# Byshx/Poccala

Measured on AMD Instinct MI355X. Metric: frames/sec GMM-score+fwd-bwd, 39-d MFCC, 2048-mix, higher is better.
Workload: dtype f32-class (f16x2 split operands, f32 accumulate; f64 dynamic programming)

## Files before the change

poccala_amd/csrc/gmm_score_split.hip:

```cpp
#include <stdlib.h>

#include "pcl_internal.h"

namespace {

#ifndef PCL_SPLIT_WG
#define PCL_SPLIT_WG 256
#endif
constexpr int WG = PCL_SPLIT_WG;
typedef float f16v __attribute__((ext_vector_type(16)));

#ifndef PCL_SPLIT16_NT
#define PCL_SPLIT16_NT 2
#endif
#ifndef PCL_SPLIT16_MINW
#define PCL_SPLIT16_MINW 3
#endif
#ifndef PCL_SPLIT16_MTS
#define PCL_SPLIT16_MTS 1
#endif
typedef _Float16 h8v __attribute__((ext_vector_type(8)));

template <int D, int NT>
__global__ __launch_bounds__(WG, PCL_SPLIT16_MINW * 256 / WG > 0 ? PCL_SPLIT16_MINW * 256 / WG : 1) void gmm_score_split16_kernel(
    const float *__restrict__ frames, const uint4 *__restrict__ pm, const float *__restrict__ fscale, const float *__restrict__ centers,
    int nmt_max, const ScoreTile *__restrict__ tiles, const ScoreSeg *__restrict__ segs, double *__restrict__ out,
    int *__restrict__ flags, const double *__restrict__ kzero, const int *__restrict__ n_on_pipe, const int *__restrict__ npt) {
    static_assert(D % 8 != 0, "the folded constants need a spare slot");
    constexpr int KS8 = (D + 7) / 8;
    constexpr int CH = 2 * KS8;
    constexpr int SC = D / 8, JC = D % 8;
    constexpr float FMAXH = 6.0e4f;
    const ScoreTile tile = tiles[blockIdx.x];
    const int lane = threadIdx.x & 63;
    const int wave = threadIdx.x >> 6;
    const int half = lane >> 5;
    const int col = lane & 31;
    if (tile.seg_lo >= tile.seg_hi) {
        if (threadIdx.x == 0) flags[blockIdx.x] = 0;
        return;
    }
    const int n_mtiles = npt[tile.state];
    __shared__ int s_ovf;
    if (threadIdx.x == 0) s_ovf = 0;
    __syncthreads();
    const int vend = segs[tile.seg_hi - 1].vstart + segs[tile.seg_hi - 1].len;
    const bool wave_active = tile.vstart + wave * NT * 32 < vend;
    if (n_mtiles == 0) {
        if (wave_active) {
            for (int c = 0; c < NT; ++c) {
                const int v = tile.vstart + (wave * NT + c) * 32 + col;
                if (v < vend && half == 0) {
                    int lo = tile.seg0;
                    const int hi = tile.seg_hi - 1;
                    while (lo < hi && segs[lo + 1].vstart <= v) ++lo;
                    const ScoreSeg sg = segs[lo];
                    out[sg.out0 + (long long)(v - sg.vstart) * sg.out_stride] = -INFINITY;
                }
            }
        }
        if (threadIdx.x == 0) flags[blockIdx.x] = 0;
        return;
    }

    h8v xb[NT][2][KS8];
    long long oidx[NT];
    bool valid[NT];
    const float *cen = centers + (size_t)tile.state * D;
    const float *fs = fscale + ((size_t)tile.state * 2 + half) * (KS8 * 8);
    bool ovf = false;
#pragma unroll
    for (int c = 0; c < NT; ++c) {
        int v = tile.vstart + (wave * NT + c) * 32 + col;
        valid[c] = v < vend;
        if (!valid[c]) v = tile.vstart;
        int lo = tile.seg0, hi = tile.seg_hi - 1;
        if (lo < hi && segs[lo + 1].vstart <= v) {
            ++lo;
            if (lo < hi && segs[lo + 1].vstart <= v) {
                ++lo;
                while (lo < hi) {
                    int mid = (lo + hi + 1) >> 1;
                    if (segs[mid].vstart <= v) lo = mid; else hi = mid - 1;
                }
            }
        }
        const ScoreSeg sg = segs[lo];
        const long long t = v - sg.vstart;
        const float *fp = frames + (sg.frame0 + t) * D;
#pragma unroll
        for (int s = 0; s < KS8; ++s)
#pragma unroll
            for (int j = 0; j < 8; ++j) {
                const int d = 8 * s + j;
                float val = 0.f;
                if (d < D) {
                    const float xc = fp[d] - cen[d];
                    val = (half ? xc : xc * xc) * fs[d];
                    ovf |= __builtin_fabsf(val) > FMAXH;
                    val = __builtin_fminf(__builtin_fmaxf(val, -FMAXH), FMAXH);
                }
                if (d == D) val = half ? 0.f : 1.f;
                const _Float16 h1 = (_Float16)val;
                xb[c][0][s][j] = h1;
                xb[c][1][s][j] = (_Float16)(val - (float)h1);
            }
        oidx[c] = sg.out0 + t * (long long)sg.out_stride;
    }
    if (__any(ovf) && lane == 0) s_ovf = 1;

    float sm[NT], ref[NT];
    bool inited[NT];
#pragma unroll
    for (int c = 0; c < NT; ++c) {
        sm[c] = 0.f;
        ref[c] = 0.f;
        inited[c] = false;
    }
    bool ref_ovf = false;

    constexpr int MTS = PCL_SPLIT16_MTS;
    __shared__ __attribute__((aligned(16))) uint4 abuf[2][MTS * CH * 64];
    const uint4 *pstate = pm + (size_t)tile.state * nmt_max * (CH * 64);
    auto dma = [&](int buf, int stage) {
        const uint4 *src = pstate + (size_t)stage * (MTS * CH * 64);
        const int nch = min(MTS, n_mtiles - stage * MTS) * CH;
        for (int p = wave; p < nch; p += WG / 64)
            __builtin_amdgcn_global_load_lds((const __attribute__((address_space(1))) void *)(src + p * 64 + lane),
                                             (__attribute__((address_space(3))) void *)&abuf[buf][p * 64], 16, 0, 0);
    };

#ifdef PCL_SPLIT_STAMPS
    unsigned long long st_acc[4] = {0, 0, 0, 0}, st_t = 0;
#define SSTAMP(k) { const unsigned long long t_ = __builtin_amdgcn_s_memtime(); st_acc[k] += t_ - st_t; st_t = t_; }
#else
#define SSTAMP(k)
#endif
    auto process = [&](int mt) {
        const uint4 *ab = &abuf[(mt / MTS) & 1][(mt % MTS) * (CH * 64)];
        f16v acc[NT];
#pragma unroll
        for (int c = 0; c < NT; ++c)
#pragma unroll
            for (int r = 0; r < 16; ++r) acc[c][r] = 0.f;
        auto pass = [&](int pa, int pb) {
#pragma unroll
            for (int s = 0; s < KS8; ++s) {
                const h8v a = *reinterpret_cast<const h8v *>(&ab[(pa * KS8 + s) * 64 + lane]);
#pragma unroll
                for (int c = 0; c < NT; ++c) acc[c] = __builtin_amdgcn_mfma_f32_32x32x16_f16(a, xb[c][pb][s], acc[c], 0, 0, 0);
            }
        };
#ifdef PCL_SPLIT_PRIO
        __builtin_amdgcn_s_setprio(1);
#endif
        pass(1, 0);
        pass(0, 1);
        pass(0, 0);
        SSTAMP(1)
#ifdef PCL_SPLIT_PRIO
        __builtin_amdgcn_s_setprio(0);
#endif
#ifdef PCL_DIAG_NOLSE
#pragma unroll
        for (int c = 0; c < NT; ++c) sm[c] += acc[c][0] + acc[c][15];
        return;
#endif
#pragma unroll
        for (int c = 0; c < NT; ++c) {
            float es[16];
#pragma unroll
            for (int r = 0; r < 16; ++r) es[r] = __builtin_amdgcn_exp2f(acc[c][r]);
#pragma unroll
            for (int w = 8; w >= 1; w >>= 1)
#pragma unroll
                for (int r = 0; r < w; ++r) es[r] += es[r + w];
            const float snew = sm[c] + es[0];
            if (__any(!inited[c]) || __any(!(snew < 3.0e38f))) {
                float gm = acc[c][0];
#pragma unroll
                for (int r = 1; r < 16; ++r) gm = __builtin_fmaxf(gm, acc[c][r]);
                const float gp = __builtin_fmaxf(gm, __shfl_xor(gm, 32, 64));
                float s = sm[c];
                const bool first = !inited[c];
                if ((first || gp > 0.f) && gp > -5.0e4f) {
                    const _Float16 r1 = (_Float16)__builtin_fminf(__builtin_fmaxf(-(ref[c] + gp), -FMAXH), FMAXH);
                    const float nref = -(float)r1, dl = nref - ref[c];
                    ref_ovf |= __builtin_fabsf(nref) > 5.0e4f;
#ifdef PCL_LSE_FLUSH_REPRO
                    s = first ? 0.f : s * __builtin_amdgcn_exp2f(-dl);
#else
                    const float hs = __builtin_amdgcn_exp2f(-0.5f * dl);
                    s = first ? 0.f : (s * hs) * hs;
#endif
                    inited[c] = true;
#pragma unroll
                    for (int r = 0; r < 16; ++r) acc[c][r] -= dl;
                    ref[c] = nref;
                    if (half) xb[c][0][SC][JC] = r1;
                }
#pragma unroll
                for (int r = 0; r < 16; ++r) s += __builtin_amdgcn_exp2f(acc[c][r]);
                sm[c] = s;
            } else {
                sm[c] = snew;
            }
        }
        SSTAMP(2)
    };
    const int n_stages = (n_mtiles + MTS - 1) / MTS;
    dma(0, 0);
#ifdef PCL_SPLIT_STAMPS
    st_t = __builtin_amdgcn_s_memtime();
#endif
    for (int st = 0; st < n_stages; ++st) {
        asm volatile("s_waitcnt vmcnt(0)" ::: "memory");
        SSTAMP(3)
        __syncthreads();
        SSTAMP(0)
        if (st == 0 && threadIdx.x == 0) flags[blockIdx.x] = s_ovf;
        if (st + 1 < n_stages) dma((st + 1) & 1, st + 1);
        if (wave_active) {
            const int mend = min(n_mtiles, (st + 1) * MTS);
            for (int mt = st * MTS; mt < mend; ++mt) process(mt);
        }
    }
#ifdef PCL_SPLIT_STAMPS
    if (blockIdx.x == 800 && lane == 0)
        printf("wave %d: per m-tile: dma-wait %llu  barrier %llu  dma-issue+lds+mfma %llu  lse %llu (memtime ticks)\n", wave,
               st_acc[3] / n_mtiles, st_acc[0] / n_mtiles, st_acc[1] / n_mtiles, st_acc[2] / n_mtiles);
#endif
    constexpr double LN2 = 0.693147180559945309417232121458;
    const double k0 = kzero[tile.state];
    if (wave_active && n_on_pipe[tile.state] > 0) {
#pragma unroll
        for (int c = 0; c < NT; ++c) ref_ovf |= !inited[c];
    }
#pragma unroll
    for (int c = 0; c < NT; ++c) {
        const double S = (double)sm[c] + (double)__shfl_xor(sm[c], 32, 64);
        if (valid[c] && half == 0) out[oidx[c]] = (S > 0) ? LN2 * ((double)ref[c] + k0 + ::log2(S)) : -INFINITY;
    }
    if (__any(ref_ovf) && lane == 0) s_ovf = 1;
    __syncthreads();
    if (threadIdx.x == 0 && s_ovf) flags[blockIdx.x] = 1;
}

template <int D>
void launch16_t(pcl_ctx *ctx, pcl_batch *b, const ScoreTile *tiles, int n_tiles) {
    constexpr size_t static_lds = 2 * (size_t)(2 * ((D + 7) / 8)) * 64 * 16;
    const size_t pad = (ctx->score_wgs_per_cu == 2 && static_lds < (56u << 10)) ? (56u << 10) - static_lds : 0;
    hipLaunchKernelGGL((gmm_score_split16_kernel<D, PCL_SPLIT16_NT>), dim3(n_tiles), dim3(WG), pad, ctx->stream, ctx->frames32,
                       reinterpret_cast<const uint4 *>(ctx->pm16f), ctx->fscale, ctx->centers32, ctx->Mpad32 / 32, tiles, b->d_segs,
                       b->Bt, b->d_tile_flags, ctx->kzero, ctx->d_non, ctx->d_npt);
}

}

int pcl_score_split16_tile_frames() { return WG / 64 * PCL_SPLIT16_NT * 32; }

int pcl_launch_score_split16(pcl_ctx *ctx, pcl_batch *b, const ScoreTile *tiles, int n_tiles) {
    if (n_tiles == 0) return PCL_OK;
    pcl_timer_begin(ctx, "score");
    switch (ctx->D) {
#define CASE(DD) case DD: launch16_t<DD>(ctx, b, tiles, n_tiles); break;
        PCL_MFMA_DIMS(CASE)
#undef CASE
        default: PCL_FAIL(ctx, PCL_ERR_INVALID, "internal: no split-f16 scoring kernel for D=%d", ctx->D);
    }
    pcl_timer_end(ctx, "score");
    HIPCHK(ctx, hipGetLastError());
    return PCL_OK;
}
```

Baseline: 20.75 million.

## Software-pipeline MFMA m-tiles with exp2 log-sum-exp of previous tile

Restructures the scoring loop so each step issues the MFMA chain for m-tile mt while computing exp2/log-sum-exp on the accumulators of m-tile mt-1, with sched_group_barrier interleaving MFMA and transcendental ops. It adds an optional 3-slot LDS ring using partial vmcnt waits and places the overflow flag inside the same LDS array. Launch-bounds min waves drops from 3 to 2, to make room for the doubled accumulator registers. The cost is higher VGPR pressure and lower occupancy, and the rescale path must now also shift the in-flight accumulator.

```diff
diff --git a/poccala_amd/csrc/gmm_score_split.hip b/poccala_amd/csrc/gmm_score_split.hip
--- a/poccala_amd/csrc/gmm_score_split.hip
+++ b/poccala_amd/csrc/gmm_score_split.hip
@@ -14,10 +14,13 @@
 #define PCL_SPLIT16_NT 2
 #endif
 #ifndef PCL_SPLIT16_MINW
-#define PCL_SPLIT16_MINW 3
-#endif
-#ifndef PCL_SPLIT16_MTS
-#define PCL_SPLIT16_MTS 1
+#define PCL_SPLIT16_MINW 2
+#endif
+#ifndef PCL_SPLIT16_RING
+#define PCL_SPLIT16_RING 2
+#endif
+#ifndef PCL_SPLIT16_TRANS_PER_MFMA
+#define PCL_SPLIT16_TRANS_PER_MFMA 1
 #endif
 typedef _Float16 h8v __attribute__((ext_vector_type(8)));
 
@@ -41,7 +44,9 @@
         return;
     }
     const int n_mtiles = npt[tile.state];
-    __shared__ int s_ovf;
+    constexpr int CHUNKS = 2 * ((D + 7) / 8);
+    __shared__ __attribute__((aligned(16))) uint4 lds[PCL_SPLIT16_RING * CHUNKS * 64 + 1];
+    int &s_ovf = *reinterpret_cast<int *>(&lds[PCL_SPLIT16_RING * CHUNKS * 64]);
     if (threadIdx.x == 0) s_ovf = 0;
     __syncthreads();
     const int vend = segs[tile.seg_hi - 1].vstart + segs[tile.seg_hi - 1].len;
@@ -119,67 +124,89 @@
     }
     bool ref_ovf = false;
 
-    constexpr int MTS = PCL_SPLIT16_MTS;
-    __shared__ __attribute__((aligned(16))) uint4 abuf[2][MTS * CH * 64];
+    constexpr int RING = PCL_SPLIT16_RING;
+    constexpr int NW = WG / 64;
+    uint4(*abuf)[CH * 64] = reinterpret_cast<uint4(*)[CH * 64]>(lds);
     const uint4 *pstate = pm + (size_t)tile.state * nmt_max * (CH * 64);
-    auto dma = [&](int buf, int stage) {
-        const uint4 *src = pstate + (size_t)stage * (MTS * CH * 64);
-        const int nch = min(MTS, n_mtiles - stage * MTS) * CH;
-        for (int p = wave; p < nch; p += WG / 64)
+    auto dma = [&](int slot, int mt) {
+        const uint4 *src = pstate + (size_t)mt * (CH * 64);
+        for (int p = wave; p < CH; p += NW)
             __builtin_amdgcn_global_load_lds((const __attribute__((address_space(1))) void *)(src + p * 64 + lane),
-                                             (__attribute__((address_space(3))) void *)&abuf[buf][p * 64], 16, 0, 0);
+                                             (__attribute__((address_space(3))) void *)&abuf[slot][p * 64], 16, 0, 0);
     };
-
-#ifdef PCL_SPLIT_STAMPS
-    unsigned long long st_acc[4] = {0, 0, 0, 0}, st_t = 0;
-#define SSTAMP(k) { const unsigned long long t_ = __builtin_amdgcn_s_memtime(); st_acc[k] += t_ - st_t; st_t = t_; }
-#else
-#define SSTAMP(k)
-#endif
-    auto process = [&](int mt) {
-        const uint4 *ab = &abuf[(mt / MTS) & 1][(mt % MTS) * (CH * 64)];
-        f16v acc[NT];
-#pragma unroll
-        for (int c = 0; c < NT; ++c)
-#pragma unroll
-            for (int r = 0; r < 16; ++r) acc[c][r] = 0.f;
-        auto pass = [&](int pa, int pb) {
-#pragma unroll
-            for (int s = 0; s < KS8; ++s) {
-                const h8v a = *reinterpret_cast<const h8v *>(&ab[(pa * KS8 + s) * 64 + lane]);
-#pragma unroll
-                for (int c = 0; c < NT; ++c) acc[c] = __builtin_amdgcn_mfma_f32_32x32x16_f16(a, xb[c][pb][s], acc[c], 0, 0, 0);
-            }
-        };
-#ifdef PCL_SPLIT_PRIO
-        __builtin_amdgcn_s_setprio(1);
-#endif
-        pass(1, 0);
-        pass(0, 1);
-        pass(0, 0);
-        SSTAMP(1)
-#ifdef PCL_SPLIT_PRIO
-        __builtin_amdgcn_s_setprio(0);
-#endif
-#ifdef PCL_DIAG_NOLSE
-#pragma unroll
-        for (int c = 0; c < NT; ++c) sm[c] += acc[c][0] + acc[c][15];
-        return;
-#endif
+    auto stage_ready = [&](int mt) {
+        if constexpr (RING == 2) {
+            asm volatile("s_waitcnt vmcnt(0)" ::: "memory");
+            __syncthreads();
+            if (mt + 1 < n_mtiles) dma((mt + 1) & 1, mt + 1);
+        } else {
+            constexpr int CHI = (CH + NW - 1) / NW, CLO = CH / NW;
+            if (mt + 1 >= n_mtiles) asm volatile("s_waitcnt vmcnt(0)" ::: "memory");
+            else if (CHI == CLO || wave < CH % NW) asm volatile("s_waitcnt vmcnt(%0)" ::"n"(CHI) : "memory");
+            else asm volatile("s_waitcnt vmcnt(%0)" ::"n"(CLO) : "memory");
+            asm volatile("s_waitcnt lgkmcnt(0)" ::: "memory");
+            __builtin_amdgcn_s_barrier();
+            asm volatile("" ::: "memory");
+            if (mt + 2 < n_mtiles) dma((mt + 2) % 3, mt + 2);
+        }
+    };
+
+    auto step = [&](const int mt, f16v(&an)[NT], f16v(&ac)[NT], const bool chain, const bool lse) __attribute__((always_inline)) {
+        float es[NT][16];
+        if (lse) {
+#pragma unroll
+            for (int c = 0; c < NT; ++c)
+#pragma unroll
+                for (int r = 0; r < 16; ++r) es[c][r] = __builtin_amdgcn_exp2f(ac[c][r]);
+        }
+        if (chain) {
+            const uint4 *ab = &abuf[mt % RING][0];
+#pragma unroll
+            for (int c = 0; c < NT; ++c)
+#pragma unroll
+                for (int r = 0; r < 16; ++r) an[c][r] = 0.f;
+            auto pass = [&](int pa, int pb) {
+#pragma unroll
+                for (int s = 0; s < KS8; ++s) {
+                    const h8v a = *reinterpret_cast<const h8v *>(&ab[(pa * KS8 + s) * 64 + lane]);
+#pragma unroll
+                    for (int c = 0; c < NT; ++c) an[c] = __builtin_amdgcn_mfma_f32_32x32x16_f16(a, xb[c][pb][s], an[c], 0, 0, 0);
+                }
+            };
+            pass(1, 0);
+            pass(0, 1);
+            pass(0, 0);
+        }
+        if (lse) {
+#pragma unroll
+            for (int c = 0; c < NT; ++c)
+#pragma unroll
+                for (int w = 8; w >= 1; w >>= 1)
+#pragma unroll
+                    for (int r = 0; r < w; ++r) es[c][r] += es[c][r + w];
+        }
+        if (chain && lse) {
+#pragma unroll
+            for (int i = 0; i < NT * 3 * KS8; ++i) {
+                __builtin_amdgcn_sched_group_barrier(0x008, 1, 0);
+                __builtin_amdgcn_sched_group_barrier(0x400, PCL_SPLIT16_TRANS_PER_MFMA, 0);
+                __builtin_amdgcn_sched_group_barrier(0x002, PCL_SPLIT16_TRANS_PER_MFMA, 0);
+            }
+        }
+        if (!lse) return;
+        float snew[NT];
+        bool slow[NT];
 #pragma unroll
         for (int c = 0; c < NT; ++c) {
-            float es[16];
-#pragma unroll
-            for (int r = 0; r < 16; ++r) es[r] = __builtin_amdgcn_exp2f(acc[c][r]);
-#pragma unroll
-            for (int w = 8; w >= 1; w >>= 1)
-#pragma unroll
-                for (int r = 0; r < w; ++r) es[r] += es[r + w];
-            const float snew = sm[c] + es[0];
-            if (__any(!inited[c]) || __any(!(snew < 3.0e38f))) {
-                float gm = acc[c][0];
-#pragma unroll
-                for (int r = 1; r < 16; ++r) gm = __builtin_fmaxf(gm, acc[c][r]);
+            snew[c] = sm[c] + es[c][0];
+            slow[c] = __any(!inited[c] | !(snew[c] < 3.0e38f));
+        }
+#pragma unroll
+        for (int c = 0; c < NT; ++c) {
+            if (slow[c]) {
+                float gm = ac[c][0];
+#pragma unroll
+                for (int r = 1; r < 16; ++r) gm = __builtin_fmaxf(gm, ac[c][r]);
                 const float gp = __builtin_fmaxf(gm, __shfl_xor(gm, 32, 64));
                 float s = sm[c];
                 const bool first = !inited[c];
@@ -195,41 +222,39 @@
 #endif
                     inited[c] = true;
 #pragma unroll
-                    for (int r = 0; r < 16; ++r) acc[c][r] -= dl;
+                    for (int r = 0; r < 16; ++r) ac[c][r] -= dl;
+                    if (chain) {
+#pragma unroll
+                        for (int r = 0; r < 16; ++r) an[c][r] -= dl;
+                    }
                     ref[c] = nref;
                     if (half) xb[c][0][SC][JC] = r1;
                 }
 #pragma unroll
-                for (int r = 0; r < 16; ++r) s += __builtin_amdgcn_exp2f(acc[c][r]);
+                for (int r = 0; r < 16; ++r) s += __builtin_amdgcn_exp2f(ac[c][r]);
                 sm[c] = s;
             } else {
-                sm[c] = snew;
-            }
-        }
-        SSTAMP(2)
+                sm[c] = snew[c];
+            }
+        }
     };
-    const int n_stages = (n_mtiles + MTS - 1) / MTS;
+
+    f16v acc[2][NT];
     dma(0, 0);
-#ifdef PCL_SPLIT_STAMPS
-    st_t = __builtin_amdgcn_s_memtime();
-#endif
-    for (int st = 0; st < n_stages; ++st) {
-        asm volatile("s_waitcnt vmcnt(0)" ::: "memory");
-        SSTAMP(3)
-        __syncthreads();
-        SSTAMP(0)
-        if (st == 0 && threadIdx.x == 0) flags[blockIdx.x] = s_ovf;
-        if (st + 1 < n_stages) dma((st + 1) & 1, st + 1);
+    if (RING == 3 && n_mtiles > 1) dma(1, 1);
+    stage_ready(0);
+    if (wave_active) step(0, acc[0], acc[1], true, false);
+    for (int mt = 1; mt < n_mtiles; ++mt) {
+        stage_ready(mt);
         if (wave_active) {
-            const int mend = min(n_mtiles, (st + 1) * MTS);
-            for (int mt = st * MTS; mt < mend; ++mt) process(mt);
-        }
-    }
-#ifdef PCL_SPLIT_STAMPS
-    if (blockIdx.x == 800 && lane == 0)
-        printf("wave %d: per m-tile: dma-wait %llu  barrier %llu  dma-issue+lds+mfma %llu  lse %llu (memtime ticks)\n", wave,
-               st_acc[3] / n_mtiles, st_acc[0] / n_mtiles, st_acc[1] / n_mtiles, st_acc[2] / n_mtiles);
-#endif
+            if (mt & 1) step(mt, acc[1], acc[0], true, true);
+            else step(mt, acc[0], acc[1], true, true);
+        }
+    }
+    if (wave_active) {
+        if (n_mtiles & 1) step(0, acc[1], acc[0], false, true);
+        else step(0, acc[0], acc[1], false, true);
+    }
     constexpr double LN2 = 0.693147180559945309417232121458;
     const double k0 = kzero[tile.state];
     if (wave_active && n_on_pipe[tile.state] > 0) {
@@ -243,12 +268,12 @@
     }
     if (__any(ref_ovf) && lane == 0) s_ovf = 1;
     __syncthreads();
-    if (threadIdx.x == 0 && s_ovf) flags[blockIdx.x] = 1;
+    if (threadIdx.x == 0) flags[blockIdx.x] = s_ovf;
 }
 
 template <int D>
 void launch16_t(pcl_ctx *ctx, pcl_batch *b, const ScoreTile *tiles, int n_tiles) {
-    constexpr size_t static_lds = 2 * (size_t)(2 * ((D + 7) / 8)) * 64 * 16;
+    constexpr size_t static_lds = PCL_SPLIT16_RING * (size_t)(2 * ((D + 7) / 8)) * 64 * 16 + 16;
     const size_t pad = (ctx->score_wgs_per_cu == 2 && static_lds < (56u << 10)) ? (56u << 10) - static_lds : 0;
     hipLaunchKernelGGL((gmm_score_split16_kernel<D, PCL_SPLIT16_NT>), dim3(n_tiles), dim3(WG), pad, ctx->stream, ctx->frames32,
                        reinterpret_cast<const uint4 *>(ctx->pm16f), ctx->fscale, ctx->centers32, ctx->Mpad32 / 32, tiles, b->d_segs,
```

Measured after the change: 18.84 million. -9.2%, worse.
